# XuanHuang0/VANeRF

Hardware: AMD Instinct MI355X
Metric: rendered rays/sec (64 samples/ray) + PSNR vs ref, 512x334 view (higher is better)
Workload: dtype bf16x3 (bf16 MFMA on hi+lo split operands, f32 accumulate; per-sample outputs within 3.3e-5 of the f32 kernel); 1 GPU; configs/vanerf.json eval view 512x334, 64 coarse + 64 importance samples/ray, two-hand mesh 1558 verts / 3108 faces, 1 source view 256x256, random trained-like weights; rays=171008, parallelism=single

## Files before the change

vanerf_amd/csrc/bf16x3_ring.h:

```cpp
#pragma once
#include "common.h"
#include "mfma_chain.h"

namespace vanerf {
namespace {

using namespace vanerf_chain;

typedef __bf16 bf16x8 __attribute__((ext_vector_type(8)));
typedef __bf16 bf16x2 __attribute__((ext_vector_type(2)));

struct FragB { u32x4 hi, lo; };

constexpr int RING_WAVES = 8;

template <int LEVEL> constexpr int LDS_FIRST = LEVEL == 2 ? L_HEAD1 : L_IBR;
template <int LEVEL> constexpr unsigned RES_BASE_DW = layer_offset_b(LDS_FIRST<LEVEL>, LEVEL);
template <int LEVEL> constexpr unsigned RES_DW = layer_offset_b(NUM_LAYERS, LEVEL) - layer_offset_b(LDS_FIRST<LEVEL>, LEVEL);
constexpr unsigned RING_PHASE_PIECES = 16u, RING_BYTES = 2u * RING_PHASE_PIECES * 1024u;
constexpr unsigned LDS_KPT = 0u, LDS_CTRL = 2u * PE_KPT_PER_HALF * 16u, LDS_LAT0 = 768u, LDS_RING = 1024u, LDS_RES = LDS_RING + RING_BYTES;
template <int LEVEL> constexpr unsigned LDS_BIAS = LDS_RES + RES_DW<LEVEL> * 4u;
template <int LEVEL> constexpr unsigned DYN_LDS_BYTES = LDS_BIAS<LEVEL> + (LEVEL == 2 ? BIAS_TABLE_FLOATS * 4u : 0u);
template <int LEVEL> constexpr unsigned RING_PIECES = RES_BASE_DW<LEVEL> / 256u;
template <int LEVEL> constexpr unsigned RING_STREAM_PHASES = (RING_PIECES<LEVEL> + RING_PHASE_PIECES - 1u) / RING_PHASE_PIECES;
template <int LEVEL> constexpr unsigned RING_PHASES = (RING_STREAM_PHASES<LEVEL> + 1u) / 2u * 2u;
static_assert(RING_WAVES == 8 && 2u * RING_WAVES == RING_PHASE_PIECES, "the ring's DMA schedule deals 2 pieces of a phase to each of 8 waves");
static_assert(RING_PHASES<0> * RING_PHASE_PIECES * 256u <= layer_offset_b(NUM_LAYERS), "the last phase's DMA must stay inside the stream");
static_assert(RING_PHASES<1> * RING_PHASE_PIECES * 256u <= layer_offset_b(NUM_LAYERS, 1), "the last phase's DMA must stay inside the hoisted stream");
static_assert(RING_PHASES<2> * RING_PHASE_PIECES * 256u <= layer_offset_b(NUM_LAYERS, 2), "the last phase's DMA must stay inside the lean stream");
static_assert(RING_STREAM_PHASES<1> == 31u && RING_STREAM_PHASES<2> == 27u, "the streamed parts: 486 KB hoisted, 426 KB lean");
static_assert(LDS_CTRL + 8u + 2u * 4u * RING_WAVES <= LDS_LAT0 && LDS_LAT0 + 128u <= LDS_RING, "control words / constant latent overlap their neighbours");
static_assert(DYN_LDS_BYTES<0> <= 160u * 1024u && DYN_LDS_BYTES<1> <= DYN_LDS_BYTES<0> && DYN_LDS_BYTES<2> <= 160u * 1024u,
              "key points + control words + ring + resident fragments (+ bias table) must fit the CU's 160 KB");
static_assert(LDS_BIAS<2> % 16u == 0, "the bias table is read 16 bytes at a time");
extern __shared__ __attribute__((aligned(16))) u32x4 s_dyn[];
typedef __attribute__((address_space(3))) u32x4 lds_u32x4_t;
typedef __attribute__((address_space(3))) unsigned lds_u32_t;
struct LAddr {
    unsigned w[3];
    unsigned dma_lds, dma_src;
};
__device__ __forceinline__ LAddr make_laddr(int lane, unsigned wv_uniform = 0u)
{
    LAddr a;
    a.dma_lds = LDS_RING + wv_uniform * 2048u; a.dma_src = wv_uniform * 2048u;
    a.w[0] = (unsigned)lane * 16u;
    asm volatile("" : "+v"(a.w[0]));
    a.w[1] = a.w[0] + 0x10000u; a.w[2] = a.w[0] + 0x20000u;
    asm volatile("" : "+v"(a.w[1]), "+v"(a.w[2]));
    return a;
}
template <unsigned BYTE> __device__ __forceinline__ u32x4 lds_frag(const LAddr& a)
{
    return *reinterpret_cast<const lds_u32x4_t*>((size_t)(a.w[BYTE >> 16] + (BYTE & 0xffffu)));
}
__device__ __forceinline__ lds_u32_t* lds_ctrl() { return reinterpret_cast<lds_u32_t*>((size_t)LDS_CTRL); }
template <int NB> struct RingDepthB { static constexpr int value = NB == 1 ? 1 : 2; };
template <int NB> struct RingB { FragB b[RingDepthB<NB>::value]; };

template <unsigned P> __device__ __forceinline__ void ring_dma(WRsrc rs, const LAddr& la)
{
    constexpr unsigned lds_off = (P % 2u) * RING_PHASE_PIECES * 1024u, src_off = P * RING_PHASE_PIECES * 1024u;
    unsigned keep, soff;
    asm volatile("s_mov_b32 %0, m0\n\ts_add_u32 m0, %2, %4\n\ts_add_u32 %1, %3, %5\n\ts_nop 0\n\t"
                 "buffer_load_dwordx4 %6, %7, %1 offen lds\n\tbuffer_load_dwordx4 %6, %7, %1 offen offset:1024 lds\n\ts_mov_b32 m0, %0"
                 : "=&s"(keep), "=&s"(soff)
                 : "s"(la.dma_lds), "s"(la.dma_src), "i"(lds_off), "i"(src_off), "v"(la.w[0]), "s"(rs)
                 : "memory");
}
template <int LEVEL, unsigned P> __device__ __forceinline__ void phase_begin(WRsrc rs, const LAddr& la)
{
    if constexpr (P > 0) asm volatile("s_waitcnt vmcnt(0) lgkmcnt(0)\n\ts_barrier" ::: "memory");
    ring_dma<(P + 1u) % RING_PHASES<LEVEL>>(rs, la);
}

template <int LEVEL> __device__ __forceinline__ void ring_close(WRsrc rs, const LAddr& la)
{
    if constexpr (RING_STREAM_PHASES<LEVEL> % 2u == 1u) phase_begin<LEVEL, RING_PHASES<LEVEL> - 1u>(rs, la);
}

template <int LEVEL, bool RES, unsigned DW> __device__ __forceinline__ FragB wload_blk(WRsrc rs, const LAddr& la)
{
    constexpr unsigned PHASES = RING_PHASES<LEVEL>, BASE_DW = RES_BASE_DW<LEVEL>;
    static_assert(RES == (DW >= BASE_DW), "a layer's fragments are either resident or streamed through the ring: nothing is fetched per wave");
    FragB r;
    if constexpr (RES) {
        r.hi = lds_frag<LDS_RES + (DW - BASE_DW) * 4u>(la);
        r.lo = lds_frag<LDS_RES + (DW - BASE_DW + 256u) * 4u>(la);
    } else {
        constexpr unsigned q = DW / 256u;
        static_assert(q % 2u == 0 && q + 1u < PHASES * RING_PHASE_PIECES, "block fragments are two consecutive pieces inside the streamed part");
        if constexpr (q % RING_PHASE_PIECES == 0) phase_begin<LEVEL, q / RING_PHASE_PIECES>(rs, la);
        r.hi = lds_frag<LDS_RING + (q % (2u * RING_PHASE_PIECES)) * 1024u>(la);
        r.lo = lds_frag<LDS_RING + ((q + 1u) % (2u * RING_PHASE_PIECES)) * 1024u>(la);
    }
    return r;
}

template <int LEVEL, int NB, int T, bool RES, unsigned SBASE_DW> __device__ __forceinline__ RingB<NB> ring_start_b(WRsrc rs, const LAddr& la)
{
    constexpr int D = RingDepthB<NB>::value, S = (T + 7) / 8;
    RingB<NB> r;
    static_for<D>([&](auto ic) {
        constexpr int i = decltype(ic)::value;
        if constexpr (i < S * NB) r.b[i] = wload_blk<LEVEL, RES, SBASE_DW + i * 512u>(rs, la);
    });
    __builtin_amdgcn_sched_barrier(0x000F);
    return r;
}

__device__ __forceinline__ unsigned pack_bf16(float a, float b)
{
    const bf16x2 v = {(__bf16)a, (__bf16)b};
    return __builtin_bit_cast(unsigned, v);
}

struct NoPre { template <class C> __device__ __forceinline__ void operator()(C) const {} };

template <int LEVEL, int NB, int T, bool RES, unsigned SBASE_DW, class Op, class Pre = NoPre>
__device__ __forceinline__ void run_layer_b(f32x16 (&acc)[NB], RingB<NB>& ring, WRsrc rs, const LAddr& la, Op&& operand,
                                            Pre&& pre = Pre{})
{
    constexpr int D = RingDepthB<NB>::value, S = (T + 7) / 8;
    constexpr int NCH = 4;
    auto split_pair = [&](auto sc, auto ic, u32x4& bh, u32x4& bl) {
        constexpr int s = decltype(sc)::value, i = decltype(ic)::value, t0 = 8 * s + 2 * i;
        float x0 = 0.0f, x1 = 0.0f;
        if constexpr (t0 < T) x0 = operand(std::integral_constant<int, t0>{});
        if constexpr (t0 + 1 < T) x1 = operand(std::integral_constant<int, t0 + 1>{});
        unsigned hpk = pack_bf16(x0, x1);
        asm("" : "+v"(hpk));
        bh[i] = hpk;
        bl[i] = pack_bf16(x0 - __uint_as_float(hpk << 16), x1 - __uint_as_float(hpk & 0xffff0000u));
    };
    u32x4 bh, bl;
    pre(std::integral_constant<int, 0>{});
    static_for<4>([&](auto ic) { split_pair(std::integral_constant<int, 0>{}, ic, bh, bl); });
    __builtin_amdgcn_sched_barrier(0);
    static_for<S>([&](auto sc) {
        constexpr int s = decltype(sc)::value;
        FragB a[NB];
        const bf16x8 xh = __builtin_bit_cast(bf16x8, bh), xl = __builtin_bit_cast(bf16x8, bl);
        u32x4 nh = {}, nl = {};
        static_for<NCH>([&](auto cc) {
            constexpr int c = decltype(cc)::value;
            static_for<3 * NB>([&](auto mc) {
                constexpr int m = decltype(mc)::value, ob = m / 3, pr = m % 3, idx = s * NB + ob;
                if constexpr (m * NCH / (3 * NB) == c) {
                    if constexpr (pr == 0) {
                        a[ob] = ring.b[idx % D];
                        if constexpr (idx + D < S * NB) ring.b[idx % D] = wload_blk<LEVEL, RES, SBASE_DW + (idx + D) * 512u>(rs, la);
                    }
                    const bf16x8 wh = __builtin_bit_cast(bf16x8, a[ob].hi), wl = __builtin_bit_cast(bf16x8, a[ob].lo);
                    acc[ob] = __builtin_amdgcn_mfma_f32_32x32x16_bf16(pr == 2 ? wl : wh, pr == 1 ? xl : xh, acc[ob], 0, 0, 0);
                }
            });
            if constexpr (s + 1 < S) {
                if constexpr (c == 0) pre(std::integral_constant<int, s + 1>{});
                split_pair(std::integral_constant<int, s + 1>{}, cc, nh, nl);
            }
            __builtin_amdgcn_sched_barrier(0);
        });
        bh = nh; bl = nl;
    });
}

template <int L, int NB> __device__ __forceinline__ void load_bias(int h, f32x16 (&acc)[NB])
{
    static_assert(bias_table_floats(L) == 2u * NB * 16u, "the layer has a row in the bias table");
    unsigned a = (unsigned)h * (NB * 64u) + (LDS_BIAS<2> + bias_table_offset(L) * 4u);
    asm volatile("" : "+v"(a));
#pragma unroll
    for (int ob = 0; ob < NB; ++ob)
#pragma unroll
        for (int i = 0; i < 4; ++i) {
            const u32x4 v = *reinterpret_cast<const lds_u32x4_t*>((size_t)(a + 64u * ob + 16u * i));
            acc[ob][4 * i] = __uint_as_float(v.x); acc[ob][4 * i + 1] = __uint_as_float(v.y);
            acc[ob][4 * i + 2] = __uint_as_float(v.z); acc[ob][4 * i + 3] = __uint_as_float(v.w);
        }
}

__device__ __forceinline__ int lane_id_fresh()
{
    int l;
    asm volatile("v_mbcnt_lo_u32_b32 %0, -1, 0\n\tv_mbcnt_hi_u32_b32 %0, -1, %0" : "=v"(l));
    return l;
}

__device__ __forceinline__ void block_barrier_lds() { asm volatile("s_waitcnt lgkmcnt(0)\n\ts_barrier" ::: "memory"); }

}
}
```

vanerf_amd/csrc/query_kernel.hip:

```cpp
#include <algorithm>
#include <cstdlib>
#include <type_traits>
#include <utility>

#include "common.h"
#include "mfma_chain.h"
#include "sample_math.h"
#include "bf16x3_ring.h"

using namespace vanerf;
using namespace vanerf_chain;


namespace {

constexpr int WAVES_PER_SIMD = 2;
constexpr int WAVES_PER_SIMD_SPILL = 1;
template <int MODE> constexpr int WPB = MODE == 1 ? RING_WAVES : 4;


#ifdef VANERF_STAMPS
#define STAMP(k)                                                                                  \
    do {                                                                                          \
        unsigned long long t_;                                                                    \
// ... 1 lines not shown
        asm volatile("s_memtime %0\n\ts_waitcnt lgkmcnt(0)" : "=s"(t_)::"memory");               \
        __builtin_amdgcn_sched_barrier(0);                                                        \
        phase_cycles[k] += t_ - t_prev;                                                           \
        t_prev = t_;                                                                              \
    } while (0)
constexpr int N_PHASES = 12;
#else
#define STAMP(k) do { } while (0)
#endif

struct QueryParams {
    VanerfFrame f;
    const float* w;
    unsigned wbytes;
    const float* pts;
    const float* qsdf;
    const uint8_t* qvis;
    const float* noise;
    const int32_t* knn_in;
    const int32_t* order;
    int raw;
    long long n;
    float* out;
    uint8_t* valid;
    unsigned long long* stamps;
    unsigned* queue;
    unsigned long long* short_groups;
    float wm1[4], hm1[4];
    const float* vp;
    float *xs, *aux;
    long long npad;
};

template <int MODE, int NB> struct RingSel { using type = Ring<NB>; };
template <int NB> struct RingSel<1, NB> { using type = RingB<NB>; };

struct LLane {
    int lane;
    WRsrc xs, aux;
    unsigned voff, row4;
    bool on;
};
constexpr unsigned SPILL_OFF = 0xfffffff0u;
template <int L, int t> __device__ __forceinline__ void spill_x(const LLane& la, float v)
{
    if (la.on) __builtin_amdgcn_raw_buffer_store_b32(__float_as_uint(v), la.xs, la.voff, (unsigned)(x_row_base(L) + 2 * t) * la.row4, 0);
}
template <int K> __device__ __forceinline__ void spill_aux(const LLane& la, float v)
{
    if (la.on) __builtin_amdgcn_raw_buffer_store_b32(__float_as_uint(v), la.aux, la.voff, (unsigned)(2 * K) * la.row4, 0);
}
template <bool SPILL> __device__ __forceinline__ LLane make_llane(int lane, WRsrc xs_rs, WRsrc aux_rs, long long npad, long long g, long long ngroups)
{
    LLane la;
    la.lane = lane; la.voff = SPILL_OFF; la.row4 = 0; la.on = SPILL;
    if constexpr (SPILL) {
        la.xs = xs_rs; la.aux = aux_rs;
        unsigned r4 = (unsigned)npad * 4u;
        asm volatile("" : "+s"(r4));
        la.row4 = r4;
        if (g < ngroups) la.voff = 4u * ((unsigned)g * 32u + (unsigned)(lane & 31)) + (unsigned)(lane >> 5) * r4;
    }
    return la;
}
template <int MODE> struct LaneSel { using type = LLane; };
template <> struct LaneSel<1> { using type = LAddr; };
__device__ __forceinline__ unsigned lane_of(const LLane& la) { return (unsigned)la.lane; }
template <int MODE, int LEVEL, int NB, int T, int L> __device__ __forceinline__ typename RingSel<MODE, NB>::type ring_start_m(WRsrc rs, const typename LaneSel<MODE>::type& la)
{
    if constexpr (MODE == 0) return ring_start<NB, T>(rs, layer_offset(L), lane_of(la) * NB * 4u);
    else return ring_start_b<LEVEL, NB, T, (L >= LDS_FIRST<LEVEL>), layer_offset_b(L, LEVEL)>(rs, la);
}

template <int MODE, int LEVEL, int NB, int T, int L, class Op>
__device__ __forceinline__ void run_layer_m(f32x16 (&acc)[NB], typename RingSel<MODE, NB>::type& ring, WRsrc rs, const typename LaneSel<MODE>::type& la, Op&& operand)
{
    if constexpr (MODE == 0)
        run_layer<NB, T>(acc, ring, rs, layer_offset(L), lane_of(la) * NB * 4u, [&](auto tc) -> float {
            const float b = operand(tc);
            spill_x<L, decltype(tc)::value>(la, b);
            return b;
        });
    else {
        static_assert(MODE == 0 || T == kT_b(L, LEVEL), "the kernel and the packed stream agree on the layer's k-pairs");
        run_layer_b<LEVEL, NB, T, (L >= LDS_FIRST<LEVEL>), layer_offset_b(L, LEVEL)>(acc, ring, rs, la, static_cast<Op&&>(operand));
    }
}

template <int NSTEPS, int NB, class TC> __device__ __forceinline__ float chain(const f32x16 (&src)[NB], TC, float one_h0)
{
    constexpr int t = TC::value;
    if constexpr (t < NSTEPS) return src[t / 16][t % 16];
    else return one_h0;
}
template <int MODE, int NSTEPS, int NB, class TC> __device__ __forceinline__ float chain_sp(const f32x16 (&src)[NB], TC, float one_h0)
{
    constexpr int t = TC::value;
    if constexpr (t < NSTEPS) return lazy_act<MODE, ACT_SOFTPLUS>(src[t / 16][t % 16]);
    else return one_h0;
}


struct SampleIn { float px, py, pz, sdf; int knn; unsigned char vis; };
__device__ __forceinline__ SampleIn fetch_sample(const QueryParams& P, unsigned grp, int j)
{
    const long long sr = (long long)grp * 32 + j;
    long long sc = sr < P.n ? sr : P.n - 1;
    if (P.order) sc = P.order[sc];
    SampleIn in;
    in.px = P.pts[3 * sc]; in.py = P.pts[3 * sc + 1]; in.pz = P.pts[3 * sc + 2];
    in.sdf = P.qsdf[sc]; in.knn = P.knn_in[sc]; in.vis = P.qvis[sc];
    return in;
}

__device__ __forceinline__ void key_points_to_lds(const VanerfFrame& F)
{
    if (threadIdx.x < 2 * PE_KPT_PER_HALF) s_dyn[LDS_KPT / 16 + threadIdx.x] = reinterpret_cast<const u32x4*>(F.kpt_cam)[threadIdx.x];
}
// ... 34 lines not shown
    const Bilin b0 = bilin_setup(x, y, F.h0, F.w0, P.wm1[2], P.hm1[2]);
    gather<8>(F.geo0, b0, 64, 32 * h, pix);
    if constexpr (HOIST) {
        load_row<2>(P.vp + VP_A0, (unsigned)(nn_idx * (int)VP_A0_ROW + 8 * h), a0s);
        load_row<8>(P.vp + VP_N0, (unsigned)(nn_idx * (int)VP_N0_ROW + 32 * h), nn);
        load_row<8>(P.vp + VP_T0, (unsigned)(nn_idx * (int)VP_N0_ROW + 32 * h), tw);
    } else {
        load_row<8>(F.vfeat0, (unsigned)(nn_idx * 64 + 32 * h), nn);
        load_row<8>(F.vfeat0, (unsigned)(tw_idx * 64 + 32 * h), tw);
    }
}

__device__ __forceinline__ void geo1_gathers(const QueryParams& P, float x, float y, int h, int nn_idx, int tw_idx, float (&pix8)[4], float (&nn8)[4],
                                             float (&tw8)[4])
{
    const VanerfFrame& F = P.f;
    const Bilin b1 = bilin_setup(x, y, F.h1, F.w1, P.wm1[3], P.hm1[3]);
    gather<1>(F.geo1, b1, 8, 4 * h, pix8);
    load_row<1>(F.vfeat1, (unsigned)(nn_idx * 8 + 4 * h), nn8);
    load_row<1>(F.vfeat1, (unsigned)(tw_idx * 8 + 4 * h), tw8);
}

__device__ __forceinline__ void tex_gathers(const QueryParams& P, float x, float y, const Bilin& bi, int h, int nn_idx, int tw_idx, float (&row)[32],
                                            float (&qi)[4], float (&qt)[8])
{
    const VanerfFrame& F = P.f;
    load_row<8>(F.vfeat_tex, (unsigned)((h ? tw_idx : nn_idx) * 32), row);
    gather<1>(F.img, bi, 4, 0, qi);
    const Bilin bt = bilin_setup(x, y, F.ht, F.wt, P.wm1[1], P.hm1[1]);
    gather<2>(F.tex, bt, 8, 0, qt);
}

template <int MODE, int LEVEL, int HC, int NBO, int NREG_MID, int l_at_a>
__device__ __forceinline__ void geo_scale(WRsrc W, int lane, const typename LaneSel<MODE>::type& la, typename RingSel<MODE, 1>::type& ring_at,
                                          float (&pix)[HC], float (&nn)[HC], float (&tw)[HC], float s0, float s1,
                                          f32x16 (&outacc)[NBO])
{
    constexpr int TIN = 3 * HC + 2;
    constexpr int TOUT = (NBO - 1) * 16 + NREG_MID;
    auto input = [&](auto tc) -> float {
        constexpr int t = decltype(tc)::value;
        if constexpr (t < HC) return pix[t];
        else if constexpr (t < 2 * HC) return nn[t - HC];
        else if constexpr (t < 3 * HC) return tw[t - 2 * HC];
        else if constexpr (t == 3 * HC) return s0;
        else return s1;
    };
    f32x16 at[1];
    zero<1>(at);
    run_layer_m<MODE, LEVEL, 1, TIN, l_at_a>(at, ring_at, W, la, input);
    auto r_gate = ring_start_m<MODE, LEVEL, 1, 6, l_at_a + 1>(W, la);
    auto r_mid = ring_start_m<MODE, LEVEL, NBO, TIN, l_at_a + 2>(W, la);
    if constexpr (MODE == 0) relu<1>(at);
    f32x16 gate[1];
    zero<1>(gate);
    run_layer_m<MODE, LEVEL, 1, 6, l_at_a + 1>(gate, r_gate, W, la, [&](auto tc) -> float { return lazy_act<MODE, ACT_RELU>(at[0][decltype(tc)::value]); });
    const float a0 = __shfl(sigmoid_f(gate[0][0]), lane & 31);
    const float a1 = __shfl(sigmoid_f(gate[0][1]), lane & 31);
    const float a2 = __shfl(sigmoid_f(gate[0][2]), lane & 31);
    if constexpr (MODE == 0) { constexpr int A = HC == 32 ? AUX_G0 : AUX_G1; spill_aux<A>(la, a0); spill_aux<A + 1>(la, a1); spill_aux<A + 2>(la, a2); }
#pragma unroll
    for (int t = 0; t < HC; ++t) { pix[t] *= a0; nn[t] *= a1; tw[t] *= a2; }
    if constexpr (LEVEL == 2) {
        zero<NBO>(outacc);
        run_layer_m<MODE, LEVEL, NBO, TIN, l_at_a + 2>(outacc, r_mid, W, la, input);
    } else {
        f32x16 mid[NBO];
        zero<NBO>(mid);
        run_layer_m<MODE, LEVEL, NBO, TIN, l_at_a + 2>(mid, r_mid, W, la, input);
        auto r_out = ring_start_m<MODE, LEVEL, NBO, TOUT, l_at_a + 3>(W, la);
        if constexpr (MODE == 0) relu<NBO>(mid);
        zero<NBO>(outacc);
        run_layer_m<MODE, LEVEL, NBO, TOUT, l_at_a + 3>(outacc, r_out, W, la,
                             [&](auto tc) -> float { constexpr int t = decltype(tc)::value; return lazy_act<MODE, ACT_RELU>(mid[t / 16][t % 16]); });
    }
}

template <int MODE, int LEVEL>
__device__ __forceinline__ void geo_scale0_vp(WRsrc W, int lane, const typename LaneSel<MODE>::type& la, typename RingSel<MODE, 1>::type& ring_at,
                                              float (&pix)[32], const float (&a0s)[8], const float (&n0)[32], const float (&t0)[32], float s0, float s1,
                                              f32x16 (&outacc)[2])
{
    constexpr int TIN = 32 + 2;
    auto input = [&](auto tc) -> float {
        constexpr int t = decltype(tc)::value;
        if constexpr (t < 32) return pix[t];
        else if constexpr (t == 32) return s0;
        else return s1;
    };
    f32x16 at[1];
    zero<1>(at);
#pragma unroll
    for (int r = 0; r < 8; ++r) at[0][r] = a0s[r];
    run_layer_m<MODE, LEVEL, 1, TIN, L_GEO_AT0_A>(at, ring_at, W, la, input);
    auto r_gate = ring_start_m<MODE, LEVEL, 1, 6, L_GEO_AT0_B>(W, la);
    auto r_mid = ring_start_m<MODE, LEVEL, 2, TIN, L_GEO_ATED0_A>(W, la);
    f32x16 gate[1];
    zero<1>(gate);
    run_layer_m<MODE, LEVEL, 1, 6, L_GEO_AT0_B>(gate, r_gate, W, la, [&](auto tc) -> float { return lazy_act<MODE, ACT_RELU>(at[0][decltype(tc)::value]); });
    const float a0 = __shfl(sigmoid_f(gate[0][0]), lane & 31);
    const float a1 = __shfl(sigmoid_f(gate[0][1]), lane & 31);
    const float a2 = __shfl(sigmoid_f(gate[0][2]), lane & 31);
    if constexpr (LEVEL == 2) {
#pragma unroll
        for (int t = 0; t < 32; ++t) { pix[t] *= a0; outacc[t / 16][t % 16] = fmaf(a2, t0[t], a1 * n0[t]); }
        run_layer_m<MODE, LEVEL, 2, TIN, L_GEO_ATED0_A>(outacc, r_mid, W, la, input);
    } else {
        f32x16 mid[2];
#pragma unroll
        for (int t = 0; t < 32; ++t) { pix[t] *= a0; mid[t / 16][t % 16] = fmaf(a2, t0[t], a1 * n0[t]); }
        run_layer_m<MODE, LEVEL, 2, TIN, L_GEO_ATED0_A>(mid, r_mid, W, la, input);
        auto r_out = ring_start_m<MODE, LEVEL, 2, 32, L_GEO_ATED0_B>(W, la);
        zero<2>(outacc);
        run_layer_m<MODE, LEVEL, 2, 32, L_GEO_ATED0_B>(outacc, r_out, W, la,
                             [&](auto tc) -> float { constexpr int t = decltype(tc)::value; return lazy_act<MODE, ACT_RELU>(mid[t / 16][t % 16]); });
    }
}

struct Mlp0RingF { WFrag<4> f[PE_FEATS]; };
template <int MODE> using Mlp0Ring = std::conditional_t<MODE == 0, Mlp0RingF, RingB<4>>;

template <int MODE, int LEVEL>
__device__ __forceinline__ void geo_scale1(WRsrc W, int lane, const typename LaneSel<MODE>::type& la, float (&pix8)[4], float (&nn8)[4], float (&tw8)[4],
                                           float s0, float s1, f32x16 (&g8)[1], Mlp0Ring<MODE>& ring0)
{
    auto r_at1 = ring_start_m<MODE, LEVEL, 1, 14, L_GEO_AT1_A>(W, la);
    if constexpr (MODE == 0)
        static_for<PE_FEATS>([&](auto fc) { constexpr int f = decltype(fc)::value; ring0.f[f] = wload<4>(W, (layer_offset(L_MLP0) + f * 256) * 4u, lane_of(la) * 16u); });
    geo_scale<MODE, LEVEL, 4, 1, 4, L_GEO_AT1_A>(W, lane, la, r_at1, pix8, nn8, tw8, s0, s1, g8);
    if constexpr (MODE == 1) ring0 = ring_start_b<LEVEL, 4, 180, false, layer_offset_b(L_MLP0, LEVEL)>(W, la);
}

struct Cam3 { float x, y, z; };
__device__ __forceinline__ Cam3 to_source_camera(const VanerfFrame& F, float px, float py, float pz)
{
// ... 69 lines not shown
            constexpr int t = decltype(tc)::value;
            if constexpr (t < 147) return feat[t / 7][t % 7];
            else if constexpr (LEVEL == 2 && t < 179) return lazy_act<1, ACT_RELU>(g64[(t - 147) / 16][(t - 147) % 16]);
            else return chain<32>(g64, std::integral_constant<int, t - 147>{}, one_h0);
        },
        [&](auto sc) {
            constexpr int s_ = decltype(sc)::value;
            constexpr int lo_k = s_ == 0 ? 0 : (8 * s_ - 1) / 7 + 1, hi_k = (8 * s_ + 7) / 7;
            constexpr int last_k = hi_k < PE_KPT_PER_HALF ? hi_k : PE_KPT_PER_HALF - 1;
            static_for<(last_k - lo_k + 1 < 0 ? 0 : last_k - lo_k + 1)>([&](auto dc) {
                constexpr int i = lo_k + decltype(dc)::value;
                pe_features<1>(F, kp_lds, h, c, i, feat[i]);
            });
        });
}

template <int MODE, int LEVEL>
__device__ __forceinline__ void mlp123(WRsrc W, const typename LaneSel<MODE>::type& la, int h, float one_h0, f32x16 (&a0)[4], const f32x16 (&g8)[1],
                                       f32x16 (&xv)[2])
{
    constexpr int T_MLP1 = kT_b(L_MLP1, LEVEL);
    auto r1 = ring_start_m<MODE, LEVEL, 4, T_MLP1, L_MLP1>(W, la);
    if constexpr (MODE == 0) softplus<4>(a0);
    f32x16 a1[4];
    if constexpr (LEVEL == 2) load_bias<L_MLP1, 4>(h, a1);
    else zero<4>(a1);
    run_layer_m<MODE, LEVEL, 4, T_MLP1, L_MLP1>(a1, r1, W, la, [&](auto tc) -> float { return chain_sp<MODE, 64>(a0, tc, one_h0); });
    auto r2 = ring_start_m<MODE, LEVEL, 4, 69, L_MLP2>(W, la);
    if constexpr (MODE == 0) softplus<4>(a1);
    zero<4>(a0);
    run_layer_m<MODE, LEVEL, 4, 69, L_MLP2>(a0, r2, W, la, [&](auto tc) -> float {
        constexpr int t = decltype(tc)::value;
        if constexpr (t < 64) return lazy_act<MODE, ACT_SOFTPLUS>(a1[t / 16][t % 16]);
        else if constexpr (t < 68) return LEVEL == 2 ? lazy_act<MODE, ACT_RELU>(g8[0][t - 64]) : g8[0][t - 64];
        else return one_h0;
    });
    auto r3 = ring_start_m<MODE, LEVEL, 2, 61, L_MLP3>(W, la);
    if constexpr (MODE == 0) softplus<4>(a0);
    zero<2>(xv);
    run_layer_m<MODE, LEVEL, 2, 61, L_MLP3>(xv, r3, W, la, [&](auto tc) -> float { return chain_sp<MODE, 60>(a0, tc, one_h0); });
}

template <int MODE> __device__ __forceinline__ void pool_mean_var(const typename LaneSel<MODE>::type& la, float pw, const f32x16 (&xv)[2], f32x16 (&pool)[4])
{
    if constexpr (MODE == 0)
        static_for<32>([&](auto rc) { constexpr int r = decltype(rc)::value; spill_aux<AUX_XV + r>(la, xv[r / 16][r % 16]); });
#pragma unroll
    for (int b = 0; b < 2; ++b)
#pragma unroll
        for (int r = 0; r < 16; ++r) {
            float m = pw * xv[b][r];
            float d = xv[b][r] - m;
            pool[b][r] = m;
            pool[2 + b][r] = pw * (d * d);
        }
}

template <int MODE, int LEVEL>
__device__ __forceinline__ void head_layers(WRsrc W, const typename LaneSel<MODE>::type& la, int h, float one_h0, typename RingSel<MODE, 2>::type& rh0,
                                            const f32x16 (&pool)[4], f32x16 (&head)[1])
{
    constexpr int T_HEAD0 = kT_b(L_HEAD0, LEVEL), T_HEAD1 = kT_b(L_HEAD1, LEVEL), T_HEAD2 = kT_b(L_HEAD2, LEVEL);
    f32x16 m0[2], m1[2];
    if constexpr (LEVEL == 2) load_bias<L_HEAD0, 2>(h, m0);
    else zero<2>(m0);
    run_layer_m<MODE, LEVEL, 2, T_HEAD0, L_HEAD0>(m0, rh0, W, la, [&](auto tc) -> float { return chain<64>(pool, tc, one_h0); });
    static_assert(LDS_FIRST<LEVEL> == L_HEAD2 + 1 || LDS_FIRST<LEVEL> == L_HEAD0 + 1, "the ring is closed behind its last streamed layer");
    if constexpr (MODE == 1 && LDS_FIRST<LEVEL> == L_HEAD0 + 1) ring_close<LEVEL>(W, la);
    auto rh1 = ring_start_m<MODE, LEVEL, 2, T_HEAD1, L_HEAD1>(W, la);
    if constexpr (MODE == 0) softplus<2>(m0);
    if constexpr (LEVEL == 2) load_bias<L_HEAD1, 2>(h, m1);
    else zero<2>(m1);
    run_layer_m<MODE, LEVEL, 2, T_HEAD1, L_HEAD1>(m1, rh1, W, la, [&](auto tc) -> float { return chain_sp<MODE, 32>(m0, tc, one_h0); });
    auto rh2 = ring_start_m<MODE, LEVEL, 1, T_HEAD2, L_HEAD2>(W, la);
    if constexpr (MODE == 0) softplus<2>(m1);
    if constexpr (LEVEL == 2) load_bias<L_HEAD2, 1>(h, head);
    else zero<1>(head);
    run_layer_m<MODE, LEVEL, 1, T_HEAD2, L_HEAD2>(head, rh2, W, la, [&](auto tc) -> float { return chain_sp<MODE, 32>(m1, tc, one_h0); });
    if constexpr (MODE == 1 && LDS_FIRST<LEVEL> == L_HEAD2 + 1) ring_close<LEVEL>(W, la);
}

template <int MODE, int LEVEL>
__device__ __forceinline__ void ibr_compress(WRsrc W, const typename LaneSel<MODE>::type& la, int h, float one_h0, bool any_valid, const f32x16 (&pool)[4],
                                             f32x16 (&lat)[1], typename RingSel<MODE, 3>::type& r_ta)
{
    constexpr int T_IBR = kT_b(L_IBR, LEVEL), T_TEX_AT = kT_b(L_TEX_AT_A, LEVEL);
    if (MODE == 1 && !any_valid) {
        r_ta = ring_start_m<MODE, LEVEL, 3, T_TEX_AT, L_TEX_AT_A>(W, la);
        if constexpr (MODE == 1)
            static_for<16>([&](auto rc) { constexpr int r = decltype(rc)::value; lat[0][r] = __uint_as_float(reinterpret_cast<const lds_u32_t*>((size_t)LDS_LAT0)[h * 16 + r]); });
    } else {
        auto r_ibr = ring_start_m<MODE, LEVEL, 1, T_IBR, L_IBR>(W, la);
        r_ta = ring_start_m<MODE, LEVEL, 3, T_TEX_AT, L_TEX_AT_A>(W, la);
        if constexpr (LEVEL == 2) load_bias<L_IBR, 1>(h, lat);
        else zero<1>(lat);
        run_layer_m<MODE, LEVEL, 1, T_IBR, L_IBR>(lat, r_ibr, W, la, [&](auto tc) -> float { return chain<64>(pool, tc, one_h0); });
    }
}

template <int MODE, int LEVEL>
__device__ __forceinline__ void tex_vis_fusion(WRsrc W, const typename LaneSel<MODE>::type& la, const float* vp, int h, int nn_idx, float q_vis, float vis_nn,
                                               float vis_tw, float (&row)[32], const float (&qi)[4], const float (&qt)[8], const f32x16 (&lat)[1],
                                               typename RingSel<MODE, 3>::type& r_ta, f32x16 (&rgb)[1])
{
    constexpr bool HOIST = LEVEL >= 1, LEAN = LEVEL == 2;
    constexpr int T_TEX_AT = kT_b(L_TEX_AT_A, LEVEL), T_TEX = kT_b(L_TEX_A, LEVEL);
    float q[6];
    q[0] = h ? qt[3] : qi[0]; q[1] = h ? qt[4] : qi[1]; q[2] = h ? qt[5] : qi[2];
    q[3] = h ? qt[6] : qt[0]; q[4] = h ? qt[7] : qt[1]; q[5] = h ? (LEAN ? vis_tw : 0.0f) : qt[2];
    const float t0 = h ? vis_nn : q_vis;
    [[maybe_unused]] const float t1 = h ? 0.0f : vis_tw;
    f32x16 latg = lat[0];
    auto tex_in = [&](auto tc) -> float {
        constexpr int t = decltype(tc)::value;
        if constexpr (t < 29) return row[t];
        else if constexpr (t < 35) return q[t - 29];
        else if constexpr (t < 47) return latg[t - 35];
        else if constexpr (t == 47) return t0;
        else { static_assert(!LEAN || t < 48, "the lean stream has no (vis_twin | -) pair"); return t1; }
    };
    auto from_ta = [&](auto& ta_) { return [&](auto tc) -> float { constexpr int t = decltype(tc)::value; return lazy_act<MODE, ACT_RELU>(ta_[t / 16][t % 16]); }; };
    auto tex_at_in = [&](auto tc) -> float {
        constexpr int t = decltype(tc)::value;
        if constexpr (!HOIST) return tex_in(tc);
        else if constexpr (t < 6) return q[t];
        else if constexpr (t < 18) return latg[t - 6];
        else if constexpr (t == 18) return t0;
        else { static_assert(!LEAN || t < 19, "the lean stream has no (vis_twin | -) pair"); return t1; }
    };
    f32x16 ta[3];
    if constexpr (HOIST) load_acc<3>(vp + VP_P, (unsigned)(nn_idx * (int)VP_P_ROW + 48 * h), ta);
    else zero<3>(ta);
    run_layer_m<MODE, LEVEL, 3, T_TEX_AT, L_TEX_AT_A>(ta, r_ta, W, la, tex_at_in);
    auto r_tg = ring_start_m<MODE, LEVEL, 1, 48, L_TEX_AT_B>(W, la);
    if constexpr (MODE == 0) relu<3>(ta);
    f32x16 tg[1];
    zero<1>(tg);
    run_layer_m<MODE, LEVEL, 1, 48, L_TEX_AT_B>(tg, r_tg, W, la, from_ta(ta));
    auto r_tb = ring_start_m<MODE, LEVEL, 3, T_TEX, L_TEX_A>(W, la);
    float m0 = sigmoid_f(tg[0][0]), m1 = sigmoid_f(tg[0][1]), m2 = sigmoid_f(tg[0][2]), m3 = sigmoid_f(tg[0][3]);
    float o0 = __shfl_xor(m0, 32), o1 = __shfl_xor(m1, 32), o2 = __shfl_xor(m2, 32);
    const float gq = h ? o0 : m0;
    const float g11 = h ? o2 : m1;
    const float ggf = h ? m0 : m3;
    const float glat = h ? m1 : o1;
    if constexpr (MODE == 0) {
        spill_aux<AUX_TEX>(la, gq); spill_aux<AUX_TEX + 1>(la, g11); spill_aux<AUX_TEX + 2>(la, ggf); spill_aux<AUX_TEX + 3>(la, glat);
        static_for<12>([&](auto rc) { constexpr int r = decltype(rc)::value; spill_aux<AUX_LAT + r>(la, lat[0][r]); });
    }
#pragma unroll
    for (int t = 0; t < 11; ++t) row[t] *= g11;
#pragma unroll
    for (int t = 11; t < 29; ++t) row[t] *= ggf;
#pragma unroll
    for (int t = 0; t < (LEAN ? 5 : 6); ++t) q[t] *= gq;
    if constexpr (LEAN) q[5] = h ? q[5] : q[5] * gq;
#pragma unroll
    for (int r = 0; r < 12; ++r) latg[r] = lat[0][r] * glat;
    zero<3>(ta);
    run_layer_m<MODE, LEVEL, 3, T_TEX, L_TEX_A>(ta, r_tb, W, la, tex_in);
    auto r_rgb = ring_start_m<MODE, LEVEL, 1, 48, L_TEX_B>(W, la);
    if constexpr (MODE == 0) relu<3>(ta);
    zero<1>(rgb);
    run_layer_m<MODE, LEVEL, 1, 48, L_TEX_B>(rgb, r_rgb, W, la, from_ta(ta));
}

__device__ __forceinline__ void store_sample(const QueryParams& P, bool live, int h, long long s, float mask, const f32x16 (&head)[1], const f32x16 (&rgb)[1])
{
    if (live && h == 0) {
        float rad = head[0][1];
        if (P.noise) rad += P.noise[s];
        float* o = P.out + 5 * s;
        o[0] = P.raw ? head[0][0] : mask * fmaxf(rad, 0.0f);
        o[1] = P.raw ? head[0][1] : mask * head[0][0] + (1.0f - mask) * P.f.invalid_sdf;
        o[2] = rgb[0][0];
        o[3] = rgb[0][1];
        o[4] = rgb[0][2];
        if (P.valid) P.valid[s] = mask > 0.0f;
    }
}

template <int MODE, bool SPILL = false, int LEVEL = 0>
__global__ __launch_bounds__(64 * WPB<MODE>, SPILL ? WAVES_PER_SIMD_SPILL : WAVES_PER_SIMD) void query_kernel(const QueryParams P)
{
    static_assert(!SPILL || MODE == 0, "the training spill runs on the fp32 kernel");
    static_assert(LEVEL >= 0 && LEVEL <= 2 && (LEVEL == 0 || MODE == 1), "only the split-bf16 kernel has a hoisted and a lean variant");
    constexpr bool HOIST = LEVEL >= 1;
    constexpr int WAVES_PER_BLOCK = WPB<MODE>;
    const int lane_k = threadIdx.x & 63;
    [[maybe_unused]] const int lane = lane_k, j = lane & 31;
    [[maybe_unused]] const long long wave = (long long)blockIdx.x * WAVES_PER_BLOCK + (threadIdx.x >> 6);
    const long long ngroups = (P.n + 31) / 32;
    const VanerfFrame& F = P.f;
    const WRsrc W = __builtin_amdgcn_make_buffer_rsrc(const_cast<float*>(P.w), 0, P.wbytes, 0x00020000);
    [[maybe_unused]] WRsrc xs_rs = W, aux_rs = W;
    if constexpr (SPILL) {
        xs_rs = __builtin_amdgcn_make_buffer_rsrc(P.xs, 0, (unsigned)(X_ROWS * 4ll * P.npad), 0x00020000);
        aux_rs = __builtin_amdgcn_make_buffer_rsrc(P.aux, 0, (unsigned)(AUX_ROWS * 4ll * P.npad), 0x00020000);
    }
#ifdef VANERF_STAMPS
    unsigned long long phase_cycles[N_PHASES] = {};
    unsigned long long t_prev, rt0;
    asm volatile("s_memrealtime %0\n\ts_waitcnt lgkmcnt(0)" : "=s"(rt0)::"memory");
    asm volatile("s_memtime %0\n\ts_waitcnt lgkmcnt(0)" : "=s"(t_prev)::"memory");
#endif
    if constexpr (MODE == 1) key_points_to_lds(F);
    unsigned short_groups = 0;
    __shared__ unsigned s_ctrl0[MODE == 0 ? 2 + 2 * WAVES_PER_BLOCK : 1];
    auto s_base = [&](unsigned i) -> auto& { if constexpr (MODE == 0) return s_ctrl0[i]; else return lds_ctrl()[i]; };
    auto s_valid = [&](unsigned pp, unsigned k) -> auto& { if constexpr (MODE == 0) return s_ctrl0[2 + pp * WAVES_PER_BLOCK + k]; else return lds_ctrl()[2 + pp * WAVES_PER_BLOCK + k]; };
    const unsigned wv = threadIdx.x >> 6;
    [[maybe_unused]] const unsigned wv_u = (unsigned)__builtin_amdgcn_readfirstlane((int)wv);
    unsigned pending = 0, par = 1;
    if (threadIdx.x == 0) s_base(0) = atomicAdd(P.queue, (unsigned)WAVES_PER_BLOCK);
    if constexpr (MODE == 1) fill_lds<LEVEL>(P, W, lane, wv_u);
    __syncthreads();
    if constexpr (MODE == 1) {
        short_path_latent<LEVEL>(W, lane, wv_u);
        __syncthreads();
    }
    unsigned base_cur = s_base(0);
    if (threadIdx.x == 0) pending = atomicAdd(P.queue, (unsigned)WAVES_PER_BLOCK);
    SampleIn in_next = fetch_sample(P, base_cur + wv, j);
    while (base_cur < (unsigned)ngroups) {
        const long long g = (long long)base_cur + wv;
        const SampleIn in = in_next;
        const int lane = MODE == 1 ? lane_id_fresh() : lane_k, j = lane & 31, h = lane >> 5;
        const float one_h0 = h ? 0.0f : 1.0f;
        typename LaneSel<MODE>::type la;
        [[maybe_unused]] unsigned kp_lds = 0;
        if constexpr (MODE == 1) { la = make_laddr(lane, wv_u); kp_lds = LDS_KPT + ((la.w[0] >> 9) & 1u) * (PE_KPT_PER_HALF * 16u); }
        else la = make_llane<SPILL>(lane, xs_rs, aux_rs, P.npad, g, ngroups);
        const long long s_raw = g * 32 + j;
        const bool live = s_raw < P.n;
        long long s = live ? s_raw : P.n - 1;
        if (P.order) s = P.order[s];
        const float px = in.px, py = in.py, pz = in.pz;
        const float q_sdf = in.sdf;
        const float q_vis = in.vis ? 1.0f : 0.0f;
        const Projected pr = project_and_mask(F, P.wm1[0], P.hm1[0], px, py, pz);
        const float x = pr.x, y = pr.y, mask = pr.mask;
        const bool wave_valid = __builtin_amdgcn_ballot_w64(mask > 0.0f) != 0ull;
        if (lane == 0) s_valid(par, wv) = wave_valid ? 1u : 0u;
        if (threadIdx.x == 0) s_base(par) = pending;
        block_barrier_lds();
        const unsigned base_next = (unsigned)__builtin_amdgcn_readfirstlane((int)s_base(par));
        unsigned anyv = 0;
#pragma unroll
        for (int k = 0; k < WAVES_PER_BLOCK; ++k) anyv |= s_valid(par, k);
        const bool any_valid = SPILL || __builtin_amdgcn_readfirstlane((int)anyv) != 0;
        par ^= 1u;
        if (threadIdx.x == 0) pending = atomicAdd(P.queue, (unsigned)WAVES_PER_BLOCK);
        in_next = fetch_sample(P, base_next + wv, j);
        base_cur = base_next;
        __builtin_amdgcn_sched_barrier(0x000F);
        const Bilin bi = bilin_setup(x, y, F.hi, F.wi, P.wm1[0], P.hm1[0]);
        const float pw = boundary_weight(pr);
        if constexpr (MODE == 0) spill_aux<AUX_PW>(la, pw);
        STAMP(0);
        const int nn_idx = in.knn;
        const int tw_idx = nn_idx >= VANERF_NV_HAND ? nn_idx - VANERF_NV_HAND : nn_idx + VANERF_NV_HAND;
        const float vis_nn = ld_off<float>(F.vert_vis, 4u * nn_idx), vis_tw = ld_off<float>(F.vert_vis, 4u * tw_idx);
        const float sc0 = h ? q_vis : q_sdf;
        const float sc1 = h ? vis_tw : vis_nn;
// ... 178 lines not shown
```

Measured before the change: 12.49 million rays/s.

## Stack hi and lo weight rows into one MFMA for narrow lean-kernel layers

For the lean kernel's eight layers with at most 16 output rows, each lane reads its A fragment from an offset that puts the hi weight rows in the upper M half and the lo rows in the lower half. One 32x32 MFMA then computes W_hi·x and W_lo·x together, and the two row halves are summed afterwards, cutting the bf16x3 products from three to two per k-step. It also halves the LDS fragment reads for these layers. In exchange it adds an extra VGPR for the stacked offset, extra adds after each layer, and depends on the stacked LDS layout lining up with the hi/lo pieces.

```diff
diff --git a/vanerf_amd/csrc/bf16x3_ring.h b/vanerf_amd/csrc/bf16x3_ring.h
--- a/vanerf_amd/csrc/bf16x3_ring.h
+++ b/vanerf_amd/csrc/bf16x3_ring.h
@@ -1,4 +1,6 @@
 #pragma once
+#include <type_traits>
+
 #include "common.h"
 #include "mfma_chain.h"
 
@@ -11,6 +13,8 @@
 typedef __bf16 bf16x2 __attribute__((ext_vector_type(2)));
 
 struct FragB { u32x4 hi, lo; };
+template <bool STACK> using FragOf = std::conditional_t<STACK, u32x4, FragB>;
+constexpr unsigned STACK_DELTA = 1024u - 16u * 16u;
 
 constexpr int RING_WAVES = 8;
 
@@ -39,8 +43,9 @@
 struct LAddr {
     unsigned w[3];
     unsigned dma_lds, dma_src;
+    unsigned stk;
 };
-__device__ __forceinline__ LAddr make_laddr(int lane, unsigned wv_uniform = 0u)
+__device__ __forceinline__ LAddr make_laddr(int lane, unsigned wv_uniform = 0u, bool stacked = false)
 {
     LAddr a;
     a.dma_lds = LDS_RING + wv_uniform * 2048u; a.dma_src = wv_uniform * 2048u;
@@ -48,15 +53,24 @@
     asm volatile("" : "+v"(a.w[0]));
     a.w[1] = a.w[0] + 0x10000u; a.w[2] = a.w[0] + 0x20000u;
     asm volatile("" : "+v"(a.w[1]), "+v"(a.w[2]));
+    a.stk = 0u;
+    if (stacked) {
+        a.stk = ((unsigned)lane & 16u) ? STACK_DELTA : 0u;
+        asm volatile("" : "+v"(a.stk));
+    }
     return a;
 }
 template <unsigned BYTE> __device__ __forceinline__ u32x4 lds_frag(const LAddr& a)
 {
     return *reinterpret_cast<const lds_u32x4_t*>((size_t)(a.w[BYTE >> 16] + (BYTE & 0xffffu)));
+}
+template <unsigned BYTE> __device__ __forceinline__ u32x4 lds_frag_stacked(const LAddr& a)
+{
+    return *reinterpret_cast<const lds_u32x4_t*>((size_t)(a.w[BYTE >> 16] + a.stk + (BYTE & 0xffffu)));
 }
 __device__ __forceinline__ lds_u32_t* lds_ctrl() { return reinterpret_cast<lds_u32_t*>((size_t)LDS_CTRL); }
 template <int NB> struct RingDepthB { static constexpr int value = NB == 1 ? 1 : 2; };
-template <int NB> struct RingB { FragB b[RingDepthB<NB>::value]; };
+template <int NB, bool STACK = false> struct RingB { FragOf<STACK> b[RingDepthB<NB>::value]; };
 
 template <unsigned P> __device__ __forceinline__ void ring_dma(WRsrc rs, const LAddr& la)
 {
@@ -79,31 +93,41 @@
     if constexpr (RING_STREAM_PHASES<LEVEL> % 2u == 1u) phase_begin<LEVEL, RING_PHASES<LEVEL> - 1u>(rs, la);
 }
 
-template <int LEVEL, bool RES, unsigned DW> __device__ __forceinline__ FragB wload_blk(WRsrc rs, const LAddr& la)
+template <int LEVEL, bool RES, unsigned DW, bool STACK = false> __device__ __forceinline__ FragOf<STACK> wload_blk(WRsrc rs, const LAddr& la)
 {
     constexpr unsigned PHASES = RING_PHASES<LEVEL>, BASE_DW = RES_BASE_DW<LEVEL>;
     static_assert(RES == (DW >= BASE_DW), "a layer's fragments are either resident or streamed through the ring: nothing is fetched per wave");
-    FragB r;
+    static_assert(!STACK || LEVEL == 2, "only the lean kernel stacks the hi and lo rows of its narrow layers");
+    FragOf<STACK> r;
     if constexpr (RES) {
-        r.hi = lds_frag<LDS_RES + (DW - BASE_DW) * 4u>(la);
-        r.lo = lds_frag<LDS_RES + (DW - BASE_DW + 256u) * 4u>(la);
+        if constexpr (STACK) r = lds_frag_stacked<LDS_RES + (DW - BASE_DW) * 4u>(la);
+        else {
+            r.hi = lds_frag<LDS_RES + (DW - BASE_DW) * 4u>(la);
+            r.lo = lds_frag<LDS_RES + (DW - BASE_DW + 256u) * 4u>(la);
+        }
     } else {
         constexpr unsigned q = DW / 256u;
         static_assert(q % 2u == 0 && q + 1u < PHASES * RING_PHASE_PIECES, "block fragments are two consecutive pieces inside the streamed part");
+        static_assert(q % (2u * RING_PHASE_PIECES) + 1u < 2u * RING_PHASE_PIECES, "hi and lo piece lie in the same half of the ring");
         if constexpr (q % RING_PHASE_PIECES == 0) phase_begin<LEVEL, q / RING_PHASE_PIECES>(rs, la);
-        r.hi = lds_frag<LDS_RING + (q % (2u * RING_PHASE_PIECES)) * 1024u>(la);
-        r.lo = lds_frag<LDS_RING + ((q + 1u) % (2u * RING_PHASE_PIECES)) * 1024u>(la);
+        if constexpr (STACK) r = lds_frag_stacked<LDS_RING + (q % (2u * RING_PHASE_PIECES)) * 1024u>(la);
+        else {
+            r.hi = lds_frag<LDS_RING + (q % (2u * RING_PHASE_PIECES)) * 1024u>(la);
+            r.lo = lds_frag<LDS_RING + ((q + 1u) % (2u * RING_PHASE_PIECES)) * 1024u>(la);
+        }
     }
     return r;
 }
 
-template <int LEVEL, int NB, int T, bool RES, unsigned SBASE_DW> __device__ __forceinline__ RingB<NB> ring_start_b(WRsrc rs, const LAddr& la)
+template <int LEVEL, int NB, int T, bool RES, unsigned SBASE_DW, bool STACK = false>
+__device__ __forceinline__ RingB<NB, STACK> ring_start_b(WRsrc rs, const LAddr& la)
 {
     constexpr int D = RingDepthB<NB>::value, S = (T + 7) / 8;
-    RingB<NB> r;
+    static_assert(!STACK || NB == 1, "a stacked fragment is the one block of its layer");
+    RingB<NB, STACK> r;
     static_for<D>([&](auto ic) {
         constexpr int i = decltype(ic)::value;
-        if constexpr (i < S * NB) r.b[i] = wload_blk<LEVEL, RES, SBASE_DW + i * 512u>(rs, la);
+        if constexpr (i < S * NB) r.b[i] = wload_blk<LEVEL, RES, SBASE_DW + i * 512u, STACK>(rs, la);
     });
     __builtin_amdgcn_sched_barrier(0x000F);
     return r;
@@ -117,11 +141,13 @@
 
 struct NoPre { template <class C> __device__ __forceinline__ void operator()(C) const {} };
 
-template <int LEVEL, int NB, int T, bool RES, unsigned SBASE_DW, class Op, class Pre = NoPre>
-__device__ __forceinline__ void run_layer_b(f32x16 (&acc)[NB], RingB<NB>& ring, WRsrc rs, const LAddr& la, Op&& operand,
+template <int LEVEL, int NB, int T, bool RES, unsigned SBASE_DW, bool STACK = false, class Op, class Pre = NoPre>
+__device__ __forceinline__ void run_layer_b(f32x16 (&acc)[NB], RingB<NB, STACK>& ring, WRsrc rs, const LAddr& la, Op&& operand,
                                             Pre&& pre = Pre{})
 {
     constexpr int D = RingDepthB<NB>::value, S = (T + 7) / 8;
+    constexpr int NPROD = STACK ? 2 : 3;
+    static_assert(!STACK || NB == 1, "a stacked fragment is the one block of its layer");
     constexpr int NCH = 4;
     auto split_pair = [&](auto sc, auto ic, u32x4& bh, u32x4& bl) {
         constexpr int s = decltype(sc)::value, i = decltype(ic)::value, t0 = 8 * s + 2 * i;
@@ -139,20 +165,24 @@
     __builtin_amdgcn_sched_barrier(0);
     static_for<S>([&](auto sc) {
         constexpr int s = decltype(sc)::value;
-        FragB a[NB];
+        FragOf<STACK> a[NB];
         const bf16x8 xh = __builtin_bit_cast(bf16x8, bh), xl = __builtin_bit_cast(bf16x8, bl);
         u32x4 nh = {}, nl = {};
         static_for<NCH>([&](auto cc) {
             constexpr int c = decltype(cc)::value;
-            static_for<3 * NB>([&](auto mc) {
-                constexpr int m = decltype(mc)::value, ob = m / 3, pr = m % 3, idx = s * NB + ob;
-                if constexpr (m * NCH / (3 * NB) == c) {
+            static_for<NPROD * NB>([&](auto mc) {
+                constexpr int m = decltype(mc)::value, ob = m / NPROD, pr = m % NPROD, idx = s * NB + ob;
+                if constexpr (m * NCH / (NPROD * NB) == c) {
                     if constexpr (pr == 0) {
                         a[ob] = ring.b[idx % D];
-                        if constexpr (idx + D < S * NB) ring.b[idx % D] = wload_blk<LEVEL, RES, SBASE_DW + (idx + D) * 512u>(rs, la);
+                        if constexpr (idx + D < S * NB) ring.b[idx % D] = wload_blk<LEVEL, RES, SBASE_DW + (idx + D) * 512u, STACK>(rs, la);
                     }
-                    const bf16x8 wh = __builtin_bit_cast(bf16x8, a[ob].hi), wl = __builtin_bit_cast(bf16x8, a[ob].lo);
-                    acc[ob] = __builtin_amdgcn_mfma_f32_32x32x16_bf16(pr == 2 ? wl : wh, pr == 1 ? xl : xh, acc[ob], 0, 0, 0);
+                    if constexpr (STACK) {
+                        acc[ob] = __builtin_amdgcn_mfma_f32_32x32x16_bf16(__builtin_bit_cast(bf16x8, a[ob]), pr == 1 ? xl : xh, acc[ob], 0, 0, 0);
+                    } else {
+                        const bf16x8 wh = __builtin_bit_cast(bf16x8, a[ob].hi), wl = __builtin_bit_cast(bf16x8, a[ob].lo);
+                        acc[ob] = __builtin_amdgcn_mfma_f32_32x32x16_bf16(pr == 2 ? wl : wh, pr == 1 ? xl : xh, acc[ob], 0, 0, 0);
+                    }
                 }
             });
             if constexpr (s + 1 < S) {
@@ -180,6 +210,8 @@
         }
 }
 
+template <bool STACK> __device__ __forceinline__ float stacked_row(const f32x16& acc, int r) { if constexpr (STACK) return acc[r] + acc[r + 8]; else return acc[r]; }
+
 __device__ __forceinline__ int lane_id_fresh()
 {
     int l;
diff --git a/vanerf_amd/csrc/query_kernel.hip b/vanerf_amd/csrc/query_kernel.hip
--- a/vanerf_amd/csrc/query_kernel.hip
+++ b/vanerf_amd/csrc/query_kernel.hip
@@ -57,8 +57,14 @@
     long long npad;
 };
 
-template <int MODE, int NB> struct RingSel { using type = Ring<NB>; };
-template <int NB> struct RingSel<1, NB> { using type = RingB<NB>; };
+template <int MODE, int NB, bool STACK = false> struct RingSel { using type = Ring<NB>; };
+template <int NB, bool STACK> struct RingSel<1, NB, STACK> { using type = RingB<NB, STACK>; };
+constexpr bool stacked_layer(int mode, int level, int l) { return mode == 1 && level == 2 && kNB[l] == 1 && kNOUT[l] <= 16; }
+static_assert(stacked_layer(1, 2, L_GEO_AT0_A) && stacked_layer(1, 2, L_GEO_AT0_B) && stacked_layer(1, 2, L_GEO_AT1_A) && stacked_layer(1, 2, L_GEO_AT1_B) &&
+              stacked_layer(1, 2, L_GEO_ATED1_A) && stacked_layer(1, 2, L_HEAD2) && stacked_layer(1, 2, L_TEX_AT_B) && stacked_layer(1, 2, L_TEX_B) &&
+              !stacked_layer(1, 2, L_IBR) && !stacked_layer(1, 1, L_HEAD2) && !stacked_layer(0, 0, L_HEAD2),
+              "eight narrow layers of the lean kernel; ibr_compress has 24 rows and every other kernel keeps three products");
+template <int MODE, int LEVEL, int L> using LayerRing = typename RingSel<MODE, kNB[L], stacked_layer(MODE, LEVEL, L)>::type;
 
 struct LLane {
     int lane;
@@ -91,14 +97,15 @@
 template <int MODE> struct LaneSel { using type = LLane; };
 template <> struct LaneSel<1> { using type = LAddr; };
 __device__ __forceinline__ unsigned lane_of(const LLane& la) { return (unsigned)la.lane; }
-template <int MODE, int LEVEL, int NB, int T, int L> __device__ __forceinline__ typename RingSel<MODE, NB>::type ring_start_m(WRsrc rs, const typename LaneSel<MODE>::type& la)
-{
+template <int MODE, int LEVEL, int NB, int T, int L> __device__ __forceinline__ LayerRing<MODE, LEVEL, L> ring_start_m(WRsrc rs, const typename LaneSel<MODE>::type& la)
+{
+    static_assert(NB == kNB[L], "the kernel and layer_spec.h agree on the layer's output blocks");
     if constexpr (MODE == 0) return ring_start<NB, T>(rs, layer_offset(L), lane_of(la) * NB * 4u);
-    else return ring_start_b<LEVEL, NB, T, (L >= LDS_FIRST<LEVEL>), layer_offset_b(L, LEVEL)>(rs, la);
+    else return ring_start_b<LEVEL, NB, T, (L >= LDS_FIRST<LEVEL>), layer_offset_b(L, LEVEL), stacked_layer(MODE, LEVEL, L)>(rs, la);
 }
 
 template <int MODE, int LEVEL, int NB, int T, int L, class Op>
-__device__ __forceinline__ void run_layer_m(f32x16 (&acc)[NB], typename RingSel<MODE, NB>::type& ring, WRsrc rs, const typename LaneSel<MODE>::type& la, Op&& operand)
+__device__ __forceinline__ void run_layer_m(f32x16 (&acc)[NB], LayerRing<MODE, LEVEL, L>& ring, WRsrc rs, const typename LaneSel<MODE>::type& la, Op&& operand)
 {
     if constexpr (MODE == 0)
         run_layer<NB, T>(acc, ring, rs, layer_offset(L), lane_of(la) * NB * 4u, [&](auto tc) -> float {
@@ -108,7 +115,7 @@
         });
     else {
         static_assert(MODE == 0 || T == kT_b(L, LEVEL), "the kernel and the packed stream agree on the layer's k-pairs");
-        run_layer_b<LEVEL, NB, T, (L >= LDS_FIRST<LEVEL>), layer_offset_b(L, LEVEL)>(acc, ring, rs, la, static_cast<Op&&>(operand));
+        run_layer_b<LEVEL, NB, T, (L >= LDS_FIRST<LEVEL>), layer_offset_b(L, LEVEL), stacked_layer(MODE, LEVEL, L)>(acc, ring, rs, la, static_cast<Op&&>(operand));
     }
 }
 
@@ -209,12 +216,14 @@
 }
 
 template <int MODE, int LEVEL, int HC, int NBO, int NREG_MID, int l_at_a>
-__device__ __forceinline__ void geo_scale(WRsrc W, int lane, const typename LaneSel<MODE>::type& la, typename RingSel<MODE, 1>::type& ring_at,
+__device__ __forceinline__ void geo_scale(WRsrc W, int lane, const typename LaneSel<MODE>::type& la, LayerRing<MODE, LEVEL, l_at_a>& ring_at,
                                           float (&pix)[HC], float (&nn)[HC], float (&tw)[HC], float s0, float s1,
                                           f32x16 (&outacc)[NBO])
 {
     constexpr int TIN = 3 * HC + 2;
     constexpr int TOUT = (NBO - 1) * 16 + NREG_MID;
+    constexpr bool STK = stacked_layer(MODE, LEVEL, l_at_a);
+    static_assert(STK == stacked_layer(MODE, LEVEL, l_at_a + 1), "`at` and the gate layer are stacked together");
     auto input = [&](auto tc) -> float {
         constexpr int t = decltype(tc)::value;
         if constexpr (t < HC) return pix[t];
@@ -231,10 +240,10 @@
     if constexpr (MODE == 0) relu<1>(at);
     f32x16 gate[1];
     zero<1>(gate);
-    run_layer_m<MODE, LEVEL, 1, 6, l_at_a + 1>(gate, r_gate, W, la, [&](auto tc) -> float { return lazy_act<MODE, ACT_RELU>(at[0][decltype(tc)::value]); });
-    const float a0 = __shfl(sigmoid_f(gate[0][0]), lane & 31);
-    const float a1 = __shfl(sigmoid_f(gate[0][1]), lane & 31);
-    const float a2 = __shfl(sigmoid_f(gate[0][2]), lane & 31);
+    run_layer_m<MODE, LEVEL, 1, 6, l_at_a + 1>(gate, r_gate, W, la, [&](auto tc) -> float { return lazy_act<MODE, ACT_RELU>(stacked_row<STK>(at[0], decltype(tc)::value)); });
+    const float a0 = __shfl(sigmoid_f(stacked_row<STK>(gate[0], 0)), lane & 31);
+    const float a1 = __shfl(sigmoid_f(stacked_row<STK>(gate[0], 1)), lane & 31);
+    const float a2 = __shfl(sigmoid_f(stacked_row<STK>(gate[0], 2)), lane & 31);
     if constexpr (MODE == 0) { constexpr int A = HC == 32 ? AUX_G0 : AUX_G1; spill_aux<A>(la, a0); spill_aux<A + 1>(la, a1); spill_aux<A + 2>(la, a2); }
 #pragma unroll
     for (int t = 0; t < HC; ++t) { pix[t] *= a0; nn[t] *= a1; tw[t] *= a2; }
@@ -254,7 +263,7 @@
 }
 
 template <int MODE, int LEVEL>
-__device__ __forceinline__ void geo_scale0_vp(WRsrc W, int lane, const typename LaneSel<MODE>::type& la, typename RingSel<MODE, 1>::type& ring_at,
+__device__ __forceinline__ void geo_scale0_vp(WRsrc W, int lane, const typename LaneSel<MODE>::type& la, LayerRing<MODE, LEVEL, L_GEO_AT0_A>& ring_at,
                                               float (&pix)[32], const float (&a0s)[8], const float (&n0)[32], const float (&t0)[32], float s0, float s1,
                                               f32x16 (&outacc)[2])
 {
@@ -265,6 +274,8 @@
         else if constexpr (t == 32) return s0;
         else return s1;
     };
+    constexpr bool STK = stacked_layer(MODE, LEVEL, L_GEO_AT0_A);
+    static_assert(STK == stacked_layer(MODE, LEVEL, L_GEO_AT0_B), "`at` and the gate layer are stacked together");
     f32x16 at[1];
     zero<1>(at);
 #pragma unroll
@@ -274,10 +285,10 @@
     auto r_mid = ring_start_m<MODE, LEVEL, 2, TIN, L_GEO_ATED0_A>(W, la);
     f32x16 gate[1];
     zero<1>(gate);
-    run_layer_m<MODE, LEVEL, 1, 6, L_GEO_AT0_B>(gate, r_gate, W, la, [&](auto tc) -> float { return lazy_act<MODE, ACT_RELU>(at[0][decltype(tc)::value]); });
-    const float a0 = __shfl(sigmoid_f(gate[0][0]), lane & 31);
-    const float a1 = __shfl(sigmoid_f(gate[0][1]), lane & 31);
-    const float a2 = __shfl(sigmoid_f(gate[0][2]), lane & 31);
+    run_layer_m<MODE, LEVEL, 1, 6, L_GEO_AT0_B>(gate, r_gate, W, la, [&](auto tc) -> float { return lazy_act<MODE, ACT_RELU>(stacked_row<STK>(at[0], decltype(tc)::value)); });
+    const float a0 = __shfl(sigmoid_f(stacked_row<STK>(gate[0], 0)), lane & 31);
+    const float a1 = __shfl(sigmoid_f(stacked_row<STK>(gate[0], 1)), lane & 31);
+    const float a2 = __shfl(sigmoid_f(stacked_row<STK>(gate[0], 2)), lane & 31);
     if constexpr (LEVEL == 2) {
 #pragma unroll
         for (int t = 0; t < 32; ++t) { pix[t] *= a0; outacc[t / 16][t % 16] = fmaf(a2, t0[t], a1 * n0[t]); }
@@ -413,7 +424,8 @@
     run_layer_m<MODE, LEVEL, 4, 69, L_MLP2>(a0, r2, W, la, [&](auto tc) -> float {
         constexpr int t = decltype(tc)::value;
         if constexpr (t < 64) return lazy_act<MODE, ACT_SOFTPLUS>(a1[t / 16][t % 16]);
-        else if constexpr (t < 68) return LEVEL == 2 ? lazy_act<MODE, ACT_RELU>(g8[0][t - 64]) : g8[0][t - 64];
+        else if constexpr (t < 68)
+            return LEVEL == 2 ? lazy_act<MODE, ACT_RELU>(stacked_row<stacked_layer(MODE, LEVEL, L_GEO_ATED1_A)>(g8[0], t - 64)) : g8[0][t - 64];
         else return one_h0;
     });
     auto r3 = ring_start_m<MODE, LEVEL, 2, 61, L_MLP3>(W, la);
@@ -458,6 +470,7 @@
     if constexpr (LEVEL == 2) load_bias<L_HEAD2, 1>(h, head);
     else zero<1>(head);
     run_layer_m<MODE, LEVEL, 1, T_HEAD2, L_HEAD2>(head, rh2, W, la, [&](auto tc) -> float { return chain_sp<MODE, 32>(m1, tc, one_h0); });
+    if constexpr (stacked_layer(MODE, LEVEL, L_HEAD2)) { head[0][0] += head[0][8]; head[0][1] += head[0][9]; }
     if constexpr (MODE == 1 && LDS_FIRST<LEVEL> == L_HEAD2 + 1) ring_close<LEVEL>(W, la);
 }
 
@@ -519,7 +532,9 @@
     zero<1>(tg);
     run_layer_m<MODE, LEVEL, 1, 48, L_TEX_AT_B>(tg, r_tg, W, la, from_ta(ta));
     auto r_tb = ring_start_m<MODE, LEVEL, 3, T_TEX, L_TEX_A>(W, la);
-    float m0 = sigmoid_f(tg[0][0]), m1 = sigmoid_f(tg[0][1]), m2 = sigmoid_f(tg[0][2]), m3 = sigmoid_f(tg[0][3]);
+    constexpr bool STK = stacked_layer(MODE, LEVEL, L_TEX_AT_B);
+    float m0 = sigmoid_f(stacked_row<STK>(tg[0], 0)), m1 = sigmoid_f(stacked_row<STK>(tg[0], 1)), m2 = sigmoid_f(stacked_row<STK>(tg[0], 2)),
+          m3 = sigmoid_f(stacked_row<STK>(tg[0], 3));
     float o0 = __shfl_xor(m0, 32), o1 = __shfl_xor(m1, 32), o2 = __shfl_xor(m2, 32);
     const float gq = h ? o0 : m0;
     const float g11 = h ? o2 : m1;
@@ -544,6 +559,7 @@
     if constexpr (MODE == 0) relu<3>(ta);
     zero<1>(rgb);
     run_layer_m<MODE, LEVEL, 1, 48, L_TEX_B>(rgb, r_rgb, W, la, from_ta(ta));
+    if constexpr (stacked_layer(MODE, LEVEL, L_TEX_B)) { rgb[0][0] += rgb[0][8]; rgb[0][1] += rgb[0][9]; rgb[0][2] += rgb[0][10]; }
 }
 
 __device__ __forceinline__ void store_sample(const QueryParams& P, bool live, int h, long long s, float mask, const f32x16 (&head)[1], const f32x16 (&rgb)[1])
@@ -610,7 +626,7 @@
         const float one_h0 = h ? 0.0f : 1.0f;
         typename LaneSel<MODE>::type la;
         [[maybe_unused]] unsigned kp_lds = 0;
-        if constexpr (MODE == 1) { la = make_laddr(lane, wv_u); kp_lds = LDS_KPT + ((la.w[0] >> 9) & 1u) * (PE_KPT_PER_HALF * 16u); }
+        if constexpr (MODE == 1) { la = make_laddr(lane, wv_u, LEVEL == 2); kp_lds = LDS_KPT + ((la.w[0] >> 9) & 1u) * (PE_KPT_PER_HALF * 16u); }
         else la = make_llane<SPILL>(lane, xs_rs, aux_rs, P.npad, g, ngroups);
         const long long s_raw = g * 32 + j;
         const bool live = s_raw < P.n;
```

Result: faster. 12.68 million rays/s, median of 6 (+1.5%).
